# Sur091/GPU-Ray-Tracing

Hardware: AMD Instinct MI355X
Metric: Mrays/s at 1920×1080 (1/2/4/8 GPUs); achieved HBM GB/s vs roofline (higher is better)
Workload: dtype f32; 1 GPU; K3 configs[2]: 1920x1080, 500 spheres, 1 spp, one progressive update per step, max_depth 1; width=1920, height=1080, spheres=500, max_depth=1, parallelism=stripes1, scan=culled, kernel=rt_tpair_kernel<2>, frame_launch=chain

## Files before the change

### gpu-ray-tracing_amd/csrc/rt_abi.cpp

```cpp
#include <hip/hip_runtime_api.h>

#include <algorithm>
#include <cmath>
#include <cstring>
#include <new>
#include <string>
#include <vector>

#include "rt_adaptive.h"
#include "rt_chain_parts.h"
#include "rt_internal.h"
#include "rt_kernels.h"
#include "rt_occlusion_cull.h"
#include "rt_selftest_roots.h"

namespace {
thread_local std::string g_last_error = "";
}

namespace rti {

rt_status fail(rt_status s, const std::string& msg) {
    g_last_error = msg;
    return s;
}

rt_status hip_fail(hipError_t e, const char* what) {
    return fail(RT_ERR_HIP, std::string(what) + ": " + hipGetErrorString(e));
}

constexpr uint32_t kMaxDim = 1u << 16;

rt_status check_image(uint32_t w, uint32_t h) {
    if (w == 0 || h == 0 || w > kMaxDim || h > kMaxDim)
        return fail(RT_ERR_INVALID_SIZE, "image size out of range (1..65536 per side)");
// ... 117 lines not shown
    ctx->occlusion_cull = on != 0;
    return RT_OK;
}

rt_status rt_occlusion_cull_stats(rt_ctx* ctx, uint64_t out[2]) {
    if (!ctx) return fail(RT_ERR_INVALID_CONTEXT, "ctx is NULL");
    if (!out) return fail(RT_ERR_INVALID_ARGUMENT, "out is NULL");
    out[0] = out[1] = 0;
    if (!ctx->cand || ctx->cand_live == 0) return RT_OK;
    DeviceGuard guard(ctx->device);
    if (!guard.ok) return fail(RT_ERR_INVALID_DEVICE, "hipSetDevice failed");
    std::vector<uint32_t> head(2 * ctx->cand_live);
    hipError_t e = hipDeviceSynchronize();
    if (e == hipSuccess)
        e = hipMemcpy2D(head.data(), 2 * sizeof(uint32_t), ctx->cand,
                        rtk::kCandStride * sizeof(float4), 2 * sizeof(uint32_t), ctx->cand_live,
                        hipMemcpyDeviceToHost);
    if (e != hipSuccess) return hip_fail(e, "hipMemcpy2D(candidate counts)");
    for (uint64_t t = 0; t < ctx->cand_live; ++t) {
        if (head[2 * t] == rtk::kCandNone) continue;
        out[0] += head[2 * t + 1];
        out[1] += head[2 * t + 1] ? 1u : 0u;
    }
    return RT_OK;
}

rt_status rt_create(int device, rt_ctx** out_ctx) {
    if (!out_ctx) return fail(RT_ERR_INVALID_ARGUMENT, "out_ctx is NULL");
    *out_ctx = nullptr;
    int n = 0;
    hipError_t e = hipGetDeviceCount(&n);
    if (e != hipSuccess) return hip_fail(e, "hipGetDeviceCount");
    if (device < 0 || device >= n) return fail(RT_ERR_INVALID_DEVICE, "no such HIP device");
    rt_ctx* ctx = new (std::nothrow) rt_ctx();
    if (!ctx) return fail(RT_ERR_NO_MEMORY, "out of host memory");
    ctx->device = device;
    *out_ctx = ctx;
    return RT_OK;
}

rt_status rt_destroy(rt_ctx* ctx) {
    if (!ctx) return fail(RT_ERR_INVALID_CONTEXT, "ctx is NULL");
    rt_status st = RT_OK;
    {
        DeviceGuard guard(ctx->device);
        if (ctx->d_geom || ctx->d_sph || ctx->cand) (void)hipDeviceSynchronize();
// ... 396 lines not shown
```

### gpu-ray-tracing_amd/csrc/rt_context.h

```cpp
#pragma once

#include <hip/hip_runtime_api.h>

#include <vector>

#include "rt_abi.h"

namespace rtc {
struct Chain;
}

struct rt_ctx {
    int device = 0;
    int scan_mode = RT_SCAN_CULLED;
    float4* d_geom = nullptr;
    float4* d_sph = nullptr;
    uint32_t capacity = 0;
    uint32_t count = 0;
    bool valid = false;
    std::vector<rt_sphere> cached;
    uint64_t scene_gen = 0;
    double scene_bound = 0.0;
    bool radii_ok = true;
    bool normal_rn = false;
    uint32_t* d_flag = nullptr;
    float4* d_hint_rs = nullptr;
    void* d_grid = nullptr;
    struct Grid {
        uint32_t nx = 0, nz = 0, nbig = 0, items = 0;
        float x0, z0, s, inv_s, ylo, yhi, cx, cy, cz, reach, m, e;
    } grid;
    float4* cand = nullptr;
    uint32_t* wg_buf = nullptr;
    uint64_t wg_cap = 0;
    uint32_t wg_pix = 0;
    uint32_t wg_parts = 0;
    uint64_t wg_builds = 0;
    uint64_t band_gen = ~0ull, band_seen_gen = ~0ull;
    uint64_t cand_tiles = 0;
    uint64_t cand_live = 0;
    std::vector<unsigned char> cand_key;
    uint64_t cand_gen = 0;
    bool occlusion_cull = true;
    uint32_t* tile_cost = nullptr;
    uint32_t* tile_order = nullptr;
    uint64_t order_tiles = 0;
    uint64_t chain_raster_key[2] = {0, 0};
    uint64_t cost_gen = ~0ull;
    uint32_t cost_frames = 0;
    uint64_t order_gen = ~0ull;
    uint32_t order_frames = 0;
    uint32_t cost_group = 1;
    uint32_t cost_key[6] = {};
    bool cost_key_ok = false;
    uint32_t* d_band_src = nullptr;
    std::vector<uint32_t> band_src;
    int tile_order_mode = RT_TILE_ORDER_AUTO;
    float* d_srgb = nullptr;
    uint32_t* d_hx = nullptr;
    uint32_t hx_len = 0, hy_len = 0;
    struct CountRecord {
        const void* image;
        uint32_t w, h, first, step, bands, n;
    };
    std::vector<CountRecord> counts;
    uint32_t frames_per_launch = 0;
// ... 32 lines not shown
```

### gpu-ray-tracing_amd/csrc/rt_frames.cpp

```cpp
#include <hip/hip_runtime_api.h>

#include <algorithm>
#include <cstdio>
#include <cstdlib>
#include <string>
#include <vector>

#include "rt_chain_parts.h"
#include "rt_internal.h"
#include "rt_kernels.h"
#ifdef RT_CALL_STAMPS
#include <chrono>
static thread_local unsigned long long g_call_stamp[8];
static void call_stamp(int i) {
    g_call_stamp[i] = (unsigned long long)std::chrono::duration_cast<std::chrono::nanoseconds>(
                          std::chrono::steady_clock::now().time_since_epoch())
                          .count();
}
#define CALL_STAMP(i) call_stamp(i)
#else
#define CALL_STAMP(i) ((void)0)
#endif

rt_status rti::chain_report(rt_ctx* ctx) {
// ... 36 lines not shown
    return RT_OK;
}

rt_status join_aux(rt_ctx* ctx, uint32_t n, hipStream_t stream) {
    hipError_t e = hipSuccess;
    for (uint32_t k = 0; e == hipSuccess && k < n; ++k) {
        e = hipEventRecord(ctx->join_ev[k], ctx->aux[k]);
        if (e == hipSuccess) e = hipStreamWaitEvent(stream, ctx->join_ev[k], 0);
    }
    return e == hipSuccess ? RT_OK : hip_fail(e, "join (hipEventRecord / hipStreamWaitEvent)");
}

void note_launch(rt_ctx* ctx, const rtk::TraceParams& p, int kernel, uint32_t frames,
                 uint32_t parts = 1u, bool aql = false) {
    ctx->last.launches += parts;
    ctx->last.queues = parts;
    ctx->last.submit = aql ? RT_SUBMIT_AQL : RT_SUBMIT_HIP;
    ctx->last.frames += frames;
    ctx->last.max_frames_per_launch = std::max(ctx->last.max_frames_per_launch, frames);
    ctx->last.normal_rn = p.normal_rn;
    ctx->last.kernel = kernel != rtk::kTraceBounce ? kernel
                       : p.compact == 3u             ? RT_KERNEL_BOUNCE_SPLIT
                                                     : RT_KERNEL_BOUNCE + (int)p.compact;
}

#ifndef RT_AQL_AUTO_MIN_TILES
#define RT_AQL_AUTO_MIN_TILES 0
#endif
#ifndef RT_AQL_AUTO_MAX_TILES
#define RT_AQL_AUTO_MAX_TILES 0
#endif
constexpr uint64_t kAqlAutoMinTiles = RT_AQL_AUTO_MIN_TILES,
                   kAqlAutoMaxTiles = RT_AQL_AUTO_MAX_TILES;
rt_status usable_chain(rt_ctx* ctx, const rtk::TraceParams& p, rtc::Chain** out) {
    *out = nullptr;
    if (ctx->update_submit == RT_SUBMIT_HIP || ctx->chain_reported) return RT_OK;
    if (ctx->update_submit == RT_SUBMIT_AUTO) {
        const uint64_t tiles = launch_tiles(p.width, p.local_bands);
        if (tiles < kAqlAutoMinTiles || tiles >= kAqlAutoMaxTiles) return RT_OK;
    }
    const bool aql = ctx->update_submit == RT_SUBMIT_AQL;
    if (!ctx->chain_tried) {
        ctx->chain_tried = true;
        rt_status st = RT_OK;
        ctx->chain = rtc::chain_create(ctx->device, &st);
        if (st != RT_OK && aql) return st;
// ... 533 lines not shown
```

### gpu-ray-tracing_amd/csrc/rt_kernels.h

```cpp
#pragma once

#include <hip/hip_runtime_api.h>
#include <stdint.h>

#include "rt_abi.h"

namespace rtk {

constexpr uint32_t kMaxFramesPerLaunch = 128;
constexpr uint32_t kLdsMaxRecords = 4096;
constexpr uint32_t kCandStride = 64;
constexpr uint32_t kCandMax = 19;
constexpr uint32_t kCandRecOff = 1;
constexpr uint32_t kCandSphOff = 21;
constexpr uint32_t kCandNone = 0xFFFFFFFFu;
static_assert(kCandRecOff + ((kCandMax + 3u) & ~3u) <= kCandSphOff, "record chunks fit");
static_assert(kCandSphOff + 2u * kCandMax <= kCandStride, "sphere records fit");
#ifndef RT_HINT_FRAMES
#define RT_HINT_FRAMES 64
#endif
constexpr uint32_t kHintFrames = RT_HINT_FRAMES;
constexpr uint32_t kHintEntries = RT_HINT_FRAMES;
constexpr uint32_t kHintRsDepth = 16;

struct TraceParams {
    const float4* in;
    float4* out;
    float4* out2;
    uint32_t store_each;
    const float4* geom;
    const float4* sph;
    uint32_t width, height, count;
    uint32_t band_first, band_step, local_bands;
    uint32_t frames;
    uint32_t reset_first;
    uint32_t lds_records;
    uint32_t cand_k;
    const float4* cand;
// ... 62 lines not shown
    return k == kTraceListPair || k == kTraceListQuad;
}
constexpr bool is_list_kernel(int k) { return k == kTraceList || is_group_kernel(k); }
#ifndef RT_WG_WAVES
#define RT_WG_WAVES 4
#endif
constexpr bool trace_ordered(int k) {
    return k == kTraceListQuad2 || k == kTraceListPair2 ||
           (is_list_kernel(k) && (is_group_kernel(k) || RT_WG_WAVES == 1));
}
constexpr uint64_t kQuadMaxTiles = 6144;
constexpr uint64_t kQuad2MaxTiles = 20000;
constexpr uint32_t hy_offset(uint32_t width) { return (width + 63u) & ~63u; }
constexpr uint32_t pack_bands(uint32_t first, uint32_t step, bool ordered) {
    return first | ((step < 0x7FFFu ? step : 0x7FFFu) << 16) | (ordered ? 1u << 31 : 0u);
}
hipError_t launch_trace(const TraceParams& p, int kernel, hipStream_t stream);
void arm_launch_events(hipEvent_t start, hipEvent_t stop);
uint32_t disarm_launch_events();
hipError_t launch_deinterleave_bands(const float4* gathered, float4* out, uint32_t width,
                                     uint32_t height, const uint32_t* band_src,
                                     hipStream_t stream);
hipError_t launch_init(float4* out, uint64_t texels, hipStream_t stream);
hipError_t launch_candidates(const TraceParams& p, float4* cand, bool occlusion,
                             hipStream_t stream);
hipError_t launch_wg_order(const float4* cand, uint32_t tiles_x, uint32_t bands, uint32_t pix,
                           uint32_t* wg_cost, uint32_t* wg_order, hipStream_t stream,
                           uint32_t parts);
inline void part_range(uint32_t n, uint32_t parts, uint32_t k, uint32_t& first, uint32_t& len) {
    first = k * (n / parts) + (k < n % parts ? k : n % parts);
    len = n / parts + (k < n % parts ? 1u : 0u);
}
uint32_t single_wg_tiles(uint32_t pix);
uint32_t single_pix();
constexpr int kChainPix1 = 0, kChainPix1Reset = 1, kChainPix = 2, kChainPixReset = 3,
              kChainGo = 4, kChainDone = 5, kChainKernels = 6;
constexpr uint32_t kHiddenArgsBytes = 256;
hipError_t chain_load_kernels();
const char* chain_kernel_symbol(int which);
uint32_t chain_args(const TraceParams& p, int kernel, const uint32_t* abort, unsigned char* out,
                    uint32_t cap, uint32_t grid[2], uint32_t* group_threads, int* which);
hipError_t launch_deinterleave(const float4* gathered, float4* out, uint32_t width,
                               uint32_t height, uint32_t nranks, uint32_t max_local_rows,
                               hipStream_t stream);
hipError_t launch_present(const float4* in, uchar4* out, uint64_t texels,
                          const float* srgb_t, hipStream_t stream);
struct AovParams {
// ... 53 lines not shown
```

### gpu-ray-tracing_amd/csrc/rt_kernels.hip

```cpp
#include <hip/hip_ext.h>
#include <hip/hip_runtime.h>

#include "rt_device.h"
#include "rt_kernels.h"

#include <cstddef>
#include <cstring>

#if defined(__HIP_DEVICE_COMPILE__) && !defined(__gfx950__)
#error "rt_kernels.hip targets gfx950 only (cache-policy bits of the sc1 hand-offs)"
#endif

namespace rtk {

using namespace rtd;

#ifndef RT_WAVE_TRACE
#define RT_WAVE_TRACE 0
#endif
#if RT_WAVE_TRACE
constexpr uint32_t kTraceWaves = 1u << 18;
__device__ unsigned long long g_wave_t[kTraceWaves][2];
__device__ unsigned g_wave_id[kTraceWaves][2];
__device__ __forceinline__ void wave_trace(int end) {
// ... 523 lines not shown
                    black[s] = blk_s;
                } else if (hit[s]) {
                    cf[s] = att;
                    dsky[s] = nd;
                    ddsky[s] = ndd;
                    black[s] = blk_s;
                }
            }
        }
    }
#pragma unroll
    for (uint32_t s = 0; s < S; ++s) {
        const v3 c = sky_w(cf[s], dsky[s], ddsky[s]);
        if (!any_other[s]) {
            asm volatile("");
            col[s] = c;
        } else {
            col[s] = black[s] ? mk(0.0f, 0.0f, 0.0f) : c;
        }
    }
    SST_V(5, col[S - 1].x);
}

template <int kPix, bool kReset, bool kChain>
__device__ __forceinline__ void single_body(
    const float4* __restrict__ a_cand, const uint32_t* __restrict__ a_hx,
    const float4* __restrict__ a_in, uint32_t a_width, uint32_t a_height, uint32_t a_bands,
    const uint32_t* __restrict__ a_order, const SingleParams& p) {
    static_assert(kPix >= 1 && kPix <= 4, "1 to 4 tiles per wave");
    constexpr uint32_t S = kPix;
    WAVE_TRACE(0);
#if RT_SSTAMPS
    sst_put(8, __builtin_amdgcn_s_memrealtime());
    sst_put(0, __builtin_amdgcn_s_memtime());
#endif
    const uint32_t lane = threadIdx.x & 63u;
    const uint32_t wave = __builtin_amdgcn_readfirstlane(threadIdx.x >> 6);
    const uint32_t tiles_x = (a_width + 7u) >> 3;
    const uint32_t aborted =
        kChain ? __builtin_amdgcn_readfirstlane(
                     __hip_atomic_load(p.abort, __ATOMIC_RELAXED, __HIP_MEMORY_SCOPE_SYSTEM))
               : 0u;
    uint32_t gx = blockIdx.x, lband = (p.lbands & 0xFFFFu) + blockIdx.y * (p.lbands >> 16);
    if (a_order) {
        const uint32_t pos = blockIdx.y * (kChain ? p.grid_x : gridDim.x) + blockIdx.x;
        const uint32_t e = __builtin_amdgcn_readfirstlane(a_order[pos]);
// ... 228 lines not shown
template <int G>
__global__ __launch_bounds__(64 * G, RT_TPAIR_MIN_WAVES) void rt_tpair_kernel(
    const float4* __restrict__ a_cand, const uint32_t* __restrict__ a_hx,
    const float4* __restrict__ a_in, uint32_t a_width, uint32_t a_height, uint32_t a_bands,
    const TraceParams p) {
    WAVE_TRACE(0);
    constexpr uint32_t S = 2, Gu = (uint32_t)G;
    static_assert(!kSingleLds<S>, "the pair sample reads its records from the candidate blocks");
    const uint32_t lane = threadIdx.x & 63u;
    const uint32_t w = __builtin_amdgcn_readfirstlane(threadIdx.x >> 6);
    const uint32_t tiles_x = (a_width + 7u) >> 3;
    const uint32_t units_x = (tiles_x + S - 1u) / S;
    uint32_t ux = blockIdx.x, lband = blockIdx.y;
    const uint32_t band_first = a_bands & 0xFFFFu, band_step = (a_bands >> 16) & 0x7FFFu;
    if (a_bands >> 31) {
        const uint32_t t =
            __builtin_amdgcn_readfirstlane(p.tile_order[blockIdx.y * gridDim.x + blockIdx.x]);
        ux = t & 0xFFFFu;
        lband = t >> 16;
    }
    const uint32_t unit = lband * units_x + ux;
    const uint32_t tx0 = ux * S;
    TileCoord tc[S];
    uint32_t ncand[S], hxy[S], tile[S];
    const float4* blk[S];
    float4 acc[S];
    uint64_t valid_m[S];
#pragma unroll
    for (uint32_t s = 0; s < S; ++s) {
        const uint32_t tx = tx0 + s;
        const bool in = tx < tiles_x;
        tile[s] = lband * tiles_x + (in ? tx : tx0);
        tc[s] = tile_coord(a_width, a_height, band_first, band_step, tx, lband, lane);
        blk[s] = a_cand + (size_t)tile[s] * kCandStride;
        ncand[s] = in ? load_cnt(a_cand, tile[s]) : 0u;
        acc[s] = a_in[tc[s].valid ? tc[s].idx : 0];
        hxy[s] = a_hx[min(tc[s].x, a_width - 1u)] ^
                 a_hx[hy_offset(a_width) + min(tc[s].y, a_height - 1u)];
        valid_m[s] = mask_ult(tc[s].x, a_width) & mask_ult(tc[s].y, a_height);
    }
    if (p.tile_cost && w == 0u && lane == 0u)
        p.tile_cost[unit] = (uint32_t)__builtin_amdgcn_s_memtime();
    const Cam cam = cam_params(p);
    const uint32_t n0 = p.hint_n[0];
    if (!p.reset_first &&
        rt_ballot((tc[0].valid && f2u(acc[0].w) != n0) || (tc[1].valid && f2u(acc[1].w) != n0)) !=
            0ull) {
        if (w < S && tx0 + w < tiles_x) {
            const float4 res = trace_pixel<kTraceListQuad, false>(
                p, cam, w ? tile[1] : tile[0], w ? ncand[1] : ncand[0], w ? tc[1] : tc[0],
                w ? hxy[1] : hxy[0], w ? acc[1] : acc[0]);
            const TileCoord& t = w ? tc[1] : tc[0];
            if (t.valid && !p.store_each) p.out[t.idx] = res;
        }
    } else {
        const uint32_t spp = p.spp;
        __shared__ float4 s_cols[2u * Gu * S * 64u];
        __shared__ float4 s_acc[S * 64u];
        if (w == 0u)
#pragma unroll
            for (uint32_t s = 0; s < S; ++s)
                s_acc[s * 64u + lane] = p.reset_first ? make_float4(0.0f, 0.0f, 0.0f, 0.0f)
                                                      : acc[s];
        const float4 zero4 = make_float4(0.0f, 0.0f, 0.0f, 0.0f);
        static_assert(kCandMax < 0x80u && kCandNone == 0xFFFFFFFFu, "a count fits a signed byte");
        const uint32_t unit_state =
            (ncand[0] & 0xFFu) | (ncand[1] & 0xFFu) << 8 | (tile[1] - tile[0]) << 16;
        for (uint32_t f = 0; f < p.frames; f += Gu) {
            const uint32_t fw = f + w;
            v3 col[S];
            const uint32_t ng = fw < p.frames ? p.hint_n[fw] : spp;
            if (ng >= spp) {
#pragma unroll
                for (uint32_t s = 0; s < S; ++s) col[s] = zero_v3_here();
            } else {
                {
                    FrameView v;
                    v.geom = p.geom;
                    v.sph = p.sph;
                    v.count = p.count;
                    v.depth = p.depth;
                    v.seed_b = p.seed_b[fw];
                    v.normal_rn = p.normal_rn;
                    v.rs = p.hint_rs[fw * p.depth];
                    uint32_t seed[S];
                    bool live[S];
                    const float4 bv[S] = {zero4, zero4};
#pragma unroll
                    for (uint32_t s = 0; s < S; ++s) {
                        seed[s] = 1u + ng + v.seed_b;
                        live[s] = tc[s].valid;
                    }
                    const float4* blkf[S];
                    uint32_t ncf[S];
                    uint32_t t0 = tile[0], st = unit_state;
                    asm volatile("" : "+s"(t0), "+s"(st));
#pragma unroll
                    for (uint32_t s = 0; s < S; ++s) {
                        const uint32_t t = t0 + (s ? st >> 16 : 0u);
                        blkf[s] = a_cand + (size_t)t * kCandStride;
                        ncf[s] = (uint32_t)((int32_t)(st << (24u - 8u * s)) >> 24);
                    }
                    single_sample<S, true>(v, cam, tc, hxy, seed, blkf, ncf, live, valid_m, bv,
                                           nullptr, col);
                }
            }
            float4* slot = s_cols + ((f / Gu) & 1u) * Gu * S * 64u;
#pragma unroll
            for (uint32_t t = 0; t < S; ++t)
                if (w != t)
                    *reinterpret_cast<f3v*>(&slot[(w * S + t) * 64u + lane]) =
                        f3v{col[t].x, col[t].y, col[t].z};
            __syncthreads();
#pragma unroll
            for (uint32_t t = 0; t < S; ++t) {
                if (w != t) continue;
#pragma unroll
                for (uint32_t j = 0; j < Gu; ++j) {
                    const uint32_t fj = f + j;
                    if (fj >= p.frames) break;
                    const uint32_t nb = p.hint_n[fj];
                    const bool acc_frame = nb < spp;
                    const float cnt = p.hint_cnt[fj];
                    float4* out = (fj & 1u) ? p.out2 : p.out;
                    const bool store = p.store_each == 2u || fj + 2u >= p.frames;
                    const float4 ca = s_acc[t * 64u + lane];
                    v3 cs = mk(ca.x, ca.y, ca.z);
// ... 691 lines not shown
        __syncthreads();
        for (uint32_t j = lane; j < m; j += 64u) {
            const uint32_t i = s_idx[j];
            s_sph[2u * j] = gsph[2u * i];
            s_sph[2u * j + 1u] = gsph[2u * i + 1u];
        }
        __syncthreads();
        for (uint32_t j = 0; j < m; ++j) {
            const float4 gj = s_rec[j];
            if (ok && !cone_misses(k, gj)) {
                if (n < K) {
                    rec[n] = gj;
                    s_own[n][lane] = gj;
                    sph[2u * n] = s_sph[2u * j];
                    sph[2u * n + 1u] = s_sph[2u * j + 1u];
                }
                ++n;
            }
        }
        __syncthreads();
    }
    if (!mine) return;
    uint32_t removed = 0;
    if (occl && ok && n <= K && n >= 2u) {
        const Lens lens = bundle_lens(p, k);
        float t_occ = __builtin_inff();
        uint32_t j_occ = kCandNone;
        for (uint32_t j = 0; j < n; ++j) {
            const OccBounds b = occ_bounds(k, lens, s_own[j][lane]);
            s_lo[j][lane] = b.lo;
            if (b.covers && b.hi < t_occ) {
                t_occ = b.hi;
                j_occ = j;
            }
        }
        if (j_occ != kCandNone) {
            uint32_t m = 0;
            for (uint32_t j = 0; j < n; ++j) {
                if (j != j_occ && s_lo[j][lane] > t_occ) continue;
                if (m != j) {
                    rec[m] = s_own[j][lane];
                    sph[2u * m] = sph[2u * j];
                    sph[2u * m + 1u] = sph[2u * j + 1u];
                }
                ++m;
            }
            removed = n - m;
            n = m;
        }
    }
    const uint32_t c = ok && n <= K ? n : kCandNone;
    if (c != kCandNone)
        for (uint32_t q = n; q < ((n + 3u) & ~3u); ++q)
            rec[q] = make_float4(0.0f, 0.0f, 0.0f, 0.0f);
    own[0] = make_float4(__uint_as_float(c), __uint_as_float(removed), 0.0f, 0.0f);
}

__global__ __launch_bounds__(256) void rt_init_kernel(float4* __restrict__ out, uint64_t n) {
    const float4 z = make_float4(0.0f, 0.0f, 0.0f, 0.0f);
    for (uint64_t i = (uint64_t)blockIdx.x * blockDim.x + threadIdx.x; i < n;
         i += (uint64_t)gridDim.x * blockDim.x)
        out[i] = z;
}

__global__ __launch_bounds__(256) void rt_deinterleave_kernel(const float4* __restrict__ g,
                                                              float4* __restrict__ out,
                                                              uint32_t width, uint32_t height,
                                                              uint32_t nranks,
                                                              uint32_t max_local_rows) {
    const uint64_t total = (uint64_t)width * height;
    for (uint64_t i = (uint64_t)blockIdx.x * blockDim.x + threadIdx.x; i < total;
         i += (uint64_t)gridDim.x * blockDim.x) {
        const uint32_t y = (uint32_t)(i / width);
        const uint32_t x = (uint32_t)(i - (uint64_t)y * width);
        const uint32_t band = y / RT_STRIPE_ROWS;
        const uint32_t rank = band % nranks;
        const uint32_t lrow = (band / nranks) * RT_STRIPE_ROWS + (y % RT_STRIPE_ROWS);
        out[i] = g[((uint64_t)rank * max_local_rows + lrow) * width + x];
// ... 336 lines not shown
    grid[0] = g.x;
    grid[1] = g.y;
    *group_threads = 64u * kSingleWg;
    *which = (one ? kChainPix1 : kChainPix) + (p.reset_first ? 1 : 0);
    return total;
}

hipError_t launch_trace(const TraceParams& p, int kernel, hipStream_t stream) {
    if (kernel == kTraceSingle) return launch_single<(int)kSinglePix>(p, stream);
    if (kernel == kTraceSingleOne) return launch_single<1>(p, stream);
    if (kernel == kTraceCulled)
        return launch_trace_as<kTraceCulled>(p, (size_t)p.lds_records * sizeof(float4), stream);
    if (kernel == kTraceList) return launch_trace_as<kTraceList>(p, 0, stream);
    if (kernel == kTraceListPair)
        return launch_trace_as<kTraceListPair>(p, group_lds_bytes<kTraceListPair>(), stream);
    if (kernel == kTraceBounce) return launch_bounce(p, stream);
    if (kernel == kTraceListQuad)
        return launch_trace_as<kTraceListQuad>(p, group_lds_bytes<kTraceListQuad>(), stream);
    if (kernel == kTraceListQuad2) return launch_tpair<4>(p, stream);
    if (kernel == kTraceListPair2) return launch_tpair<2>(p, stream);
    return launch_trace_as<kTraceExhaustive>(p, 0, stream);
}

hipError_t launch_candidates(const TraceParams& p, float4* cand, bool occlusion,
                             hipStream_t stream) {
    const uint32_t tiles_x = (p.width + 7u) >> 3;
    const dim3 grid((tiles_x + kCandBX - 1u) / kCandBX,
                    (p.local_bands + kCandBY - 1u) / kCandBY);
    if (grid.x == 0 || grid.y == 0) return hipSuccess;
    hipLaunchKernelGGL(rt_candidates_kernel, grid, dim3(64), 0, stream, p, cand,
                       occlusion ? 1u : 0u);
    return hipGetLastError();
}

uint32_t single_wg_tiles(uint32_t pix) { return kSingleWg * pix; }
uint32_t single_pix() { return kSinglePix; }

hipError_t launch_wg_order(const float4* cand, uint32_t tiles_x, uint32_t bands, uint32_t pix,
                           uint32_t* wg_cost, uint32_t* wg_order, hipStream_t stream,
                           uint32_t parts) {
    const uint32_t per = kSingleWg * pix;
    const uint32_t cols = (tiles_x + per - 1u) / per;
    const uint32_t units = cols * bands;
    if (units == 0) return hipSuccess;
    hipLaunchKernelGGL(rt_wg_cost_kernel, dim3((units + 255u) / 256u), dim3(256), 0, stream, cand,
                       tiles_x, cols, per, units, wg_cost);
    hipError_t e = hipGetLastError();
    if (e != hipSuccess) return e;
    return launch_tile_order(wg_cost, wg_order, units, cols, stream, parts);
}

hipError_t launch_init(float4* out, uint64_t texels, hipStream_t stream) {
    if (texels == 0) return hipSuccess;
    uint64_t blocks = (texels + 255u) / 256u;
// ... 101 lines not shown
```

### gpu-ray-tracing_amd/csrc/rt_occlusion.h

```cpp
#pragma once

#include "rt_trace_device.h"

namespace rtk {

__device__ __forceinline__ v3 cross3(v3 a, v3 b) {
    return mk(a.y * b.z - a.z * b.y, a.z * b.x - a.x * b.z, a.x * b.y - a.y * b.x);
}
__device__ __forceinline__ float l1(v3 v) { return fabsf(v.x) + fabsf(v.y) + fabsf(v.z); }

struct Lens {
    v3 ctr;
    float rl;
};
__device__ __forceinline__ Lens bundle_lens(const TraceParams& p, const Cone& k) {
    Lens b;
    b.ctr = mk(p.center[0], p.center[1], p.center[2]);
    float rl = 0.0f;
    if (p.defocus_angle > 0.0f) {
        const v3 du = mk(p.ddu[0], p.ddu[1], p.ddu[2]), dv = mk(p.ddv[0], p.ddv[1], p.ddv[2]);
        rl = __builtin_amdgcn_sqrtf(dot(du, du) + dot(dv, dv));
    }
    b.rl = rl * 1.001f + 1e-5f * (l1(k.apex) + l1(b.ctr));
    return b;
}

struct OccBounds {
    float lo, hi;
    bool covers;
};
__device__ __forceinline__ OccBounds occ_bounds(const Cone& k, const Lens& b, float4 g) {
    OccBounds r;
    r.lo = -__builtin_inff();
    r.hi = __builtin_inff();
    r.covers = false;
    const v3 C = mk(g.x, g.y, g.z);
    const float R2 = g.w, R = __builtin_amdgcn_sqrtf(g.w);
    const v3 v = sub(C, k.apex);
    const float at = fabsf(dot(v, k.axis)), p = len3(cross3(v, k.axis));
    const float sl = 1e-5f * (at + p + k.r_o) + 1e-6f * (l1(C) + l1(k.apex));
    const float dl_hi = p + at * k.sin_t + k.r_o + sl;
    const float dl_lo = fmaf(p, k.cos_t, -at * k.sin_t) - k.r_o - sl;
    const v3 w = sub(C, b.ctr);
    const float D = len3(w), tc = dot(w, k.axis), pc = len3(cross3(w, k.axis));
    const float sd = 1e-5f * D + 1e-6f * (l1(C) + l1(b.ctr));
    const float s_hi = D + b.rl + sd, s_lo = D - b.rl - sd;
    const bool ahead = tc * k.cos_t - pc * k.sin_t - b.rl - sd > 0.0f && s_lo > R * 1.0001f;
    if (!ahead || !__builtin_isfinite(s_hi + dl_hi + R)) return r;
    const float E = 2e-6f * fmaf(s_hi, s_hi, R2);
    const float q2 = R2 - dl_hi * dl_hi;
    const bool inside = q2 > E;
    const float err = 1e-6f * (s_hi + R) +
                      (inside ? E * __builtin_amdgcn_rsqf(q2) * 1.0001f
                              : __builtin_amdgcn_sqrtf(E) * 1.0001f);
    {
        const float dl = fminf(fmaxf(dl_lo, 0.0f), R);
        const float num = (s_lo - R) * (s_lo + R);
        const float den = __builtin_amdgcn_sqrtf(fmaf(-dl, dl, s_lo * s_lo) * 1.000001f +
                                                 1e-6f * s_lo * s_lo) +
                          __builtin_amdgcn_sqrtf(fmaxf(fmaf(-dl, dl, R2), 0.0f) + 1e-6f * R2);
        r.lo = num / den * 0.9999f - err;
    }
    if (inside) {
        const float num = (s_hi - R) * (s_hi + R);
        const float den =
            __builtin_amdgcn_sqrtf(fmaxf(fmaf(-dl_hi, dl_hi, s_hi * s_hi) - 1e-6f * s_hi * s_hi,
                                         0.0f)) +
            __builtin_amdgcn_sqrtf(fmaxf(q2 - 1e-6f * R2, 0.0f));
        const float tangent = __builtin_amdgcn_sqrtf(num);
        r.hi = fminf(num / den, tangent) * 1.0001f + err;
        r.covers = s_lo - R - err > 1.1e-3f * k.d_max && __builtin_isfinite(r.hi);
    }
    return r;
}

}
```

### gpu-ray-tracing_amd/csrc/rt_plan.cpp

```cpp
#include <hip/hip_runtime_api.h>

#include <algorithm>
#include <cmath>
#include <cstdlib>
#include <cstring>
#include <vector>

#include "rt_device.h"
#include "rt_internal.h"
#include "rt_kernels.h"

namespace rti {

int trace_kernel_for(const rt_ctx* ctx, const rtk::TraceParams& p) {
    if (ctx->scan_mode == RT_SCAN_EXHAUSTIVE) return rtk::kTraceExhaustive;
#ifndef RT_FORCE_CULLED_KERNEL
    if (p.depth <= 1u && camera_rays_bounded(ctx, p)) return rtk::kTraceList;
#endif
#ifndef RT_NO_BOUNCE_KERNEL
    if (p.depth >= 2u) return rtk::kTraceBounce;
#endif
    return rtk::kTraceCulled;
}

// ... 27 lines not shown
                                    (tpair && tiles <= rtk::kQuad2MaxTiles)));
    return quad ? (tpair ? rtk::kTraceListQuad2 : rtk::kTraceListQuad)
                : (tpair ? rtk::kTraceListPair2 : rtk::kTraceListPair);
}

UnitGrid frame_group_units(int kernel, uint32_t w, uint32_t bands) {
    const uint32_t group =
        kernel == rtk::kTraceListQuad2 || kernel == rtk::kTraceListPair2 ? 2u : 1u;
    const uint32_t units_x = (((w + 7u) >> 3) + group - 1u) / group;
    return {group, units_x, (uint64_t)units_x * bands};
}

void free_candidates(rt_ctx* ctx) {
    (void)hipFree(ctx->cand);
    ctx->cand = nullptr;
    ctx->cand_tiles = 0;
    ctx->cand_live = 0;
    ctx->cand_key.clear();
}

static rt_status ensure_candidates(rt_ctx* ctx, rtk::TraceParams& p, hipStream_t stream) {
    struct Key {
        float center[3], vul[3], pdu[3], pdv[3], ddu[3], ddv[3], defocus;
        uint32_t w, h, first, step, bands, occlusion;
        uint64_t scene;
    } key;
    std::memset(&key, 0, sizeof(key));
    std::memcpy(key.center, p.center, sizeof(key.center));
    std::memcpy(key.vul, p.vul, sizeof(key.vul));
    std::memcpy(key.pdu, p.pdu, sizeof(key.pdu));
    std::memcpy(key.pdv, p.pdv, sizeof(key.pdv));
    std::memcpy(key.ddu, p.ddu, sizeof(key.ddu));
    std::memcpy(key.ddv, p.ddv, sizeof(key.ddv));
    key.defocus = p.defocus_angle;
    key.w = p.width;
    key.h = p.height;
    key.first = p.band_first;
    key.step = p.band_step;
    key.bands = p.local_bands;
    key.scene = ctx->scene_gen;
    const bool occlusion = ctx->occlusion_cull && ctx->scene_bound <= 0x1p40 &&
                           camera_rays_bounded(ctx, p);
    key.occlusion = occlusion ? 1u : 0u;
    const unsigned char* kb = reinterpret_cast<const unsigned char*>(&key);
    const uint64_t tiles = launch_tiles(p.width, p.local_bands);
    p.cand_k = rtk::kCandMax;
    if (ctx->cand_key.size() != sizeof(key) ||
        std::memcmp(ctx->cand_key.data(), kb, sizeof(key)) != 0) {
        if (tiles > ctx->cand_tiles) {
            if (ctx->cand_tiles) {
                hipError_t e = hipStreamSynchronize(stream);
                if (e != hipSuccess) return hip_fail(e, "hipStreamSynchronize");
            }
            free_candidates(ctx);
            hipError_t e = hipMalloc(&ctx->cand, tiles * rtk::kCandStride * sizeof(float4));
            if (e != hipSuccess) {
                free_candidates(ctx);
                return hip_fail(e, "hipMalloc(candidate lists)");
            }
            ctx->cand_tiles = tiles;
        }
        hipError_t e = rtk::launch_candidates(p, ctx->cand, occlusion, stream);
        if (e != hipSuccess) return hip_fail(e, "rt_candidates_kernel launch");
        ctx->cand_key.assign(kb, kb + sizeof(key));
        ctx->cand_gen++;
        ctx->cand_live = tiles;
    }
    p.cand = ctx->cand;
    return RT_OK;
}

rt_status ensure_order_buffers(rt_ctx* ctx, uint64_t tiles, hipStream_t stream) {
    if (tiles <= ctx->order_tiles) return RT_OK;
    if (ctx->order_tiles) {
        hipError_t e = hipStreamSynchronize(stream);
        if (e != hipSuccess) return hip_fail(e, "hipStreamSynchronize");
    }
    (void)hipFree(ctx->tile_cost);
    (void)hipFree(ctx->tile_order);
    ctx->tile_cost = ctx->tile_order = nullptr;
    ctx->order_tiles = 0;
    ctx->cost_gen = ctx->order_gen = ~0ull;
    ctx->chain_raster_key[0] = 0;
    hipError_t e = hipMalloc(&ctx->tile_cost, tiles * sizeof(uint32_t));
    if (e == hipSuccess) e = hipMalloc(&ctx->tile_order, 3 * tiles * sizeof(uint32_t));
// ... 415 lines not shown
```

### gpu-ray-tracing_amd/gpu_ray_tracing/_lib.py

```python
from __future__ import annotations

import ctypes
import os
from pathlib import Path

import torch

PKG_ROOT = Path(__file__).resolve().parent.parent
LIB_PATH = PKG_ROOT / "build" / "librt_hip.so"

F = ctypes.c_float
U32 = ctypes.c_uint32


class RtError(RuntimeError):

    def __init__(self, status: int, func: str, message: str):
        super().__init__(f"{func} failed with status {status} ({STATUS_NAMES.get(status, '?')}): "
                         f"{message}")
        self.status = status


STATUS_NAMES = {
    0: "RT_OK",
# ... 97 lines not shown
    "rt_comm_group_start": (ctypes.c_int, []),
    "rt_comm_group_end": (ctypes.c_int, []),
    "rt_gather_stripes": (ctypes.c_int, [P, P, P, P, P, U32, U32, U32, P]),
    "rt_update_frames_bands": (ctypes.c_int, [P, P, P, U32, U32, P, P, P, U32, U32, P, P,
                                              ctypes.POINTER(ctypes.c_int)]),
    "rt_band_costs": (ctypes.c_int, [P, U32, U32, P, P]),
    "rt_partition_bands": (ctypes.c_int, [P, U32, U32, P]),
    "rt_deinterleave_bands": (ctypes.c_int, [P, P, P, U32, U32, U32, P, U32, P]),
    "rt_gather_bands": (ctypes.c_int, [P, P, P, P, P, U32, U32, P, U32, P]),
    "rt_set_launch_timing": (ctypes.c_int, [P, ctypes.c_int]),
    "rt_last_call_kernel_time": (ctypes.c_int, [P, ctypes.POINTER(F), ctypes.POINTER(U32)]),
}

_SIGS_CHAIN_PARTS = {
    "rt_set_chain_parts": (ctypes.c_int, [P, U32]),
    "rt_chain_schedule": (ctypes.c_int, [U32, U32, ctypes.c_int, P, U32, ctypes.POINTER(U32)]),
}

_SIGS_OCCLUSION = {
    "rt_set_occlusion_cull": (ctypes.c_int, [P, ctypes.c_int]),
    "rt_occlusion_cull_stats": (ctypes.c_int, [P, P]),
}

_SIGS_SELFTEST_ROOTS = {
    "rt_selftest_roots": (ctypes.c_int, [P, ctypes.c_uint64, P]),
}
RT_ROOTS_FAMILIES = 2
RT_ROOTS_STRATA = 4

_SIGS_AOV = {
    "rt_trace_aov": (ctypes.c_int, [P, P, U32, U32, P, P, U32, P]),
    "rt_trace_aov_bands": (ctypes.c_int, [P, P, U32, U32, P, P, P, U32, P]),
    "rt_pick": (ctypes.c_int, [P, U32, U32, U32, U32, P, P, U32, P, P]),
}
RT_AOV_MISS = 0xFFFFFFFF
AOV_PLANES = ("sphere_id", "hit", "normal", "material")


class AovPlanesC(ctypes.Structure):
    _fields_ = [("sphere_id", P), ("hit", P), ("normal", P), ("material", P)]


class PickResultC(ctypes.Structure):
    _fields_ = [("sphere_id", U32), ("t", F), ("p", F * 3), ("normal", F * 3),
                ("front_face", U32), ("color", F * 4)]

# ... 170 lines not shown
    _fields_ = [("part", U32), ("first", U32), ("frames", U32)]


class RootsTallyC(ctypes.Structure):
    _fields_ = [("mismatches", ctypes.c_uint64), ("drawn", ctypes.c_uint64),
                ("compared", ctypes.c_uint64), ("rooted", ctypes.c_uint64)]


_lib = None


def lib() -> ctypes.CDLL:
    global _lib
    if _lib is None:
        path = Path(os.environ.get("RT_HIP_LIB", LIB_PATH))
        if not path.exists():
            raise RuntimeError(f"librt_hip.so not found at {path}: build it with "
                               f"`make -C {PKG_ROOT}` (no CPU fallback exists)")
        handle = ctypes.CDLL(str(path))
        for name, (res, args) in {**_SIGS, **_SIGS_CHAIN_PARTS, **_SIGS_SELFTEST_ROOTS,
                                  **_SIGS_AOV, **_SIGS_DENOISE, **_SIGS_REPROJECT,
                                  **_SIGS_VARIANCE, **_SIGS_ADAPTIVE, **_SIGS_CONVERGE,
                                  **_SIGS_PROGRESS, **_SIGS_EDIT, **_SIGS_OCCLUSION,
                                  **_SIGS_MATTE, **_SIGS_QUERY}.items():
            if "RT_HIP_LIB" in os.environ and not hasattr(handle, name):
                continue
            fn = getattr(handle, name)
            fn.restype = res
            fn.argtypes = args
        _lib = handle
    return _lib


_fast = False


def fastcall():
    global _fast
    if _fast is False:
        _fast = None
        if "RT_HIP_LIB" not in os.environ:
            import importlib.machinery
            import importlib.util
            import sysconfig
            path = PKG_ROOT / "build" / ("_rt_fastcall" + sysconfig.get_config_var("EXT_SUFFIX"))
            if path.exists():
                lib()
                loader = importlib.machinery.ExtensionFileLoader("_rt_fastcall", str(path))
                spec = importlib.util.spec_from_file_location("_rt_fastcall", path,
                                                              loader=loader)
                mod = importlib.util.module_from_spec(spec)
                loader.exec_module(mod)
                _fast = mod
    return _fast


def exported_symbols() -> list[str]:
    return list(_SIGS)


def chain_parts_symbols() -> list[str]:
    return list(_SIGS_CHAIN_PARTS)


def occlusion_symbols() -> list[str]:
    return list(_SIGS_OCCLUSION)


def selftest_roots_symbols() -> list[str]:
    return list(_SIGS_SELFTEST_ROOTS)


def aov_symbols() -> list[str]:
    return list(_SIGS_AOV)


def denoise_symbols() -> list[str]:
    return list(_SIGS_DENOISE)


def reproject_symbols() -> list[str]:
    return list(_SIGS_REPROJECT)


def variance_symbols() -> list[str]:
    return list(_SIGS_VARIANCE)


def adaptive_symbols() -> list[str]:
    return list(_SIGS_ADAPTIVE)

# ... 30 lines not shown
```

### gpu-ray-tracing_amd/gpu_ray_tracing/compute_shader.py

```python
from __future__ import annotations

import ctypes

import numpy as np
import torch

from . import _lib
from .camera import SceneCamera
from .scene import SphereCollection

RT_STRIPE_ROWS = _lib.RT_STRIPE_ROWS
DENOISE_DEFAULTS = {"iterations": 5, "normal_power_log2": 5, "sigma_color": 1.0,
                    "sigma_position": 0.5}


REPROJECT_DEFAULTS = {"max_history": 64, "position_tolerance2": 1e-5, "lambertian_only": True}


GUIDED_DEFAULTS = {"iterations": 5, "normal_power_log2": 5, "sigma_luminance": 1.0,
                   "sigma_position": 0.5, "min_history": 4, "fallback_variance": 1.0}


ADAPTIVE_DEFAULTS = {"min_samples": 16, "abs_tolerance2": 1e-5, "rel_tolerance2": 2.5e-4}

# ... 136 lines not shown
            self._ctx = ctypes.c_void_p()

    def set_frames_per_launch(self, n: int) -> None:
        _lib.call("rt_set_frames_per_launch", self._ctx, int(n))

    def set_frame_pairs(self, mode: str) -> None:
        _lib.call("rt_set_frame_pairs", self._ctx,
                  {"auto": 0, "off": 1, "on": 2, "quad": 3, "on2": 4, "quad2": 5}[mode])

    def set_frame_images(self, mode: str) -> None:
        _lib.call("rt_set_frame_images", self._ctx, {"last_two": 0, "every": 1}[mode])

    def set_tile_order(self, mode: str) -> None:
        _lib.call("rt_set_tile_order", self._ctx, {"auto": 0, "off": 1}[mode])

    def set_update_queues(self, queues: int) -> None:
        _lib.call("rt_set_update_queues", self._ctx, int(queues))

    def set_chain_parts(self, parts: int) -> None:
        _lib.call("rt_set_chain_parts", self._ctx, int(parts))

    def set_occlusion_cull(self, on: bool) -> None:
        _lib.call("rt_set_occlusion_cull", self._ctx, 1 if on else 0)

    def set_update_submit(self, mode: str) -> None:
        _lib.call("rt_set_update_submit", self._ctx, {"auto": 0, "hip": 1, "aql": 2}[mode])

    def submit_status(self) -> dict:
        avail, give_ups, packets = ctypes.c_int(0), _lib.U32(0), ctypes.c_uint64(0)
        _lib.call("rt_update_submit_status", self._ctx, ctypes.byref(avail),
                  ctypes.byref(give_ups), ctypes.byref(packets))
        why = "" if avail.value else _lib.lib().rt_last_error().decode()
        return {"aql_available": bool(avail.value), "go_give_ups": int(give_ups.value),
                "packets": int(packets.value), "why": why}

    def set_path_compaction(self, mode: str) -> None:
        _lib.call("rt_set_path_compaction", self._ctx,
                  {"auto": 0, "per_wave": 1, "compact": 2, "pair": 3, "split": 4}[mode])

    def set_single_kernel(self, mode: str) -> None:
        _lib.call("rt_set_single_kernel", self._ctx,
                  {"auto": 0, "off": 1, "pair": 2, "one": 3}[mode])

    def frames_per_launch(self, camera) -> int:
        out = _lib.U32(0)
        cam = camera.to_c()
# ... 843 lines not shown
```

Before: 201,800 Mrays/s.

## Add certain-tile fast path skipping candidate intersection loop in pair kernel

The candidate builder now flags 8-pixel tiles where exactly one sphere remains after occlusion culling and that sphere provably covers every ray in the tile. It stores a tile-certain bit plus a material class in the tile header. The pair trace kernel packs these flags into its per-unit state. When both tiles of a pair are certain, it uses a specialised sampler that intersects that one sphere directly and shades by material class, bypassing the general candidate loop and its hit tests. This costs an extra flag load, more kernel code and registers, and a stricter coverage test in the candidate kernel. It also adds a toggle and a stats query.

```diff
diff --git a/gpu-ray-tracing_amd/csrc/rt_abi.cpp b/gpu-ray-tracing_amd/csrc/rt_abi.cpp
--- a/gpu-ray-tracing_amd/csrc/rt_abi.cpp
+++ b/gpu-ray-tracing_amd/csrc/rt_abi.cpp
@@ -11,6 +11,7 @@
 #include "rt_chain_parts.h"
 #include "rt_internal.h"
 #include "rt_kernels.h"
+#include "rt_certain_tiles.h"
 #include "rt_occlusion_cull.h"
 #include "rt_selftest_roots.h"
 
@@ -174,6 +175,37 @@
         out[0] += head[2 * t + 1];
         out[1] += head[2 * t + 1] ? 1u : 0u;
     }
+    return RT_OK;
+}
+
+rt_status rt_set_certain_tiles(rt_ctx* ctx, int on) {
+    if (!ctx) return fail(RT_ERR_INVALID_CONTEXT, "ctx is NULL");
+    if (on != 0 && on != 1) return fail(RT_ERR_INVALID_ARGUMENT, "on must be 0 or 1");
+    ctx->certain_tiles = on != 0;
+    return RT_OK;
+}
+
+rt_status rt_certain_tiles_stats(rt_ctx* ctx, uint64_t out[2]) {
+    if (!ctx) return fail(RT_ERR_INVALID_CONTEXT, "ctx is NULL");
+    if (!out) return fail(RT_ERR_INVALID_ARGUMENT, "out is NULL");
+    out[0] = out[1] = 0;
+    if (!ctx->cand || ctx->cand_live == 0 || ctx->scan_mode != RT_SCAN_CULLED) return RT_OK;
+    DeviceGuard guard(ctx->device);
+    if (!guard.ok) return fail(RT_ERR_INVALID_DEVICE, "hipSetDevice failed");
+    std::vector<uint32_t> flags(ctx->cand_live);
+    hipError_t e = hipDeviceSynchronize();
+    if (e == hipSuccess)
+        e = hipMemcpy2D(flags.data(), sizeof(uint32_t),
+                        reinterpret_cast<const uint32_t*>(ctx->cand) + 2,
+                        rtk::kCandStride * sizeof(float4), sizeof(uint32_t), ctx->cand_live,
+                        hipMemcpyDeviceToHost);
+    if (e != hipSuccess) return hip_fail(e, "hipMemcpy2D(tile flags)");
+    for (uint32_t f : flags) out[0] += f & rtk::kTileCertain;
+    const uint64_t tx = ctx->pair_tiles_x;
+    if (ctx->pair_gen == ctx->cand_gen && tx * ctx->pair_bands == ctx->cand_live)
+        for (uint64_t b = 0; b < ctx->pair_bands; ++b)
+            for (uint64_t x = 0; x + 1 < tx; x += 2)
+                out[1] += flags[b * tx + x] & flags[b * tx + x + 1] & rtk::kTileCertain;
     return RT_OK;
 }
 
diff --git a/gpu-ray-tracing_amd/csrc/rt_context.h b/gpu-ray-tracing_amd/csrc/rt_context.h
--- a/gpu-ray-tracing_amd/csrc/rt_context.h
+++ b/gpu-ray-tracing_amd/csrc/rt_context.h
@@ -42,6 +42,9 @@
     std::vector<unsigned char> cand_key;
     uint64_t cand_gen = 0;
     bool occlusion_cull = true;
+    bool certain_tiles = true;
+    uint64_t pair_gen = ~0ull;
+    uint32_t pair_tiles_x = 0, pair_bands = 0;
     uint32_t* tile_cost = nullptr;
     uint32_t* tile_order = nullptr;
     uint64_t order_tiles = 0;
diff --git a/gpu-ray-tracing_amd/csrc/rt_frames.cpp b/gpu-ray-tracing_amd/csrc/rt_frames.cpp
--- a/gpu-ray-tracing_amd/csrc/rt_frames.cpp
+++ b/gpu-ray-tracing_amd/csrc/rt_frames.cpp
@@ -82,6 +82,11 @@
     ctx->last.kernel = kernel != rtk::kTraceBounce ? kernel
                        : p.compact == 3u             ? RT_KERNEL_BOUNCE_SPLIT
                                                      : RT_KERNEL_BOUNCE + (int)p.compact;
+    if (kernel == rtk::kTraceListPair2 || kernel == rtk::kTraceListQuad2) {
+        ctx->pair_gen = ctx->cand_gen;
+        ctx->pair_tiles_x = (p.width + 7u) >> 3;
+        ctx->pair_bands = p.local_bands;
+    }
 }
 
 #ifndef RT_AQL_AUTO_MIN_TILES
diff --git a/gpu-ray-tracing_amd/csrc/rt_kernels.h b/gpu-ray-tracing_amd/csrc/rt_kernels.h
--- a/gpu-ray-tracing_amd/csrc/rt_kernels.h
+++ b/gpu-ray-tracing_amd/csrc/rt_kernels.h
@@ -14,6 +14,8 @@
 constexpr uint32_t kCandRecOff = 1;
 constexpr uint32_t kCandSphOff = 21;
 constexpr uint32_t kCandNone = 0xFFFFFFFFu;
+constexpr uint32_t kTileCertain = 1u;
+constexpr uint32_t kClassLambertian = 0u, kClassMetal = 1u, kClassDielectric = 2u;
 static_assert(kCandRecOff + ((kCandMax + 3u) & ~3u) <= kCandSphOff, "record chunks fit");
 static_assert(kCandSphOff + 2u * kCandMax <= kCandStride, "sphere records fit");
 #ifndef RT_HINT_FRAMES
@@ -122,7 +124,7 @@
                                      uint32_t height, const uint32_t* band_src,
                                      hipStream_t stream);
 hipError_t launch_init(float4* out, uint64_t texels, hipStream_t stream);
-hipError_t launch_candidates(const TraceParams& p, float4* cand, bool occlusion,
+hipError_t launch_candidates(const TraceParams& p, float4* cand, bool occlusion, bool certain,
                              hipStream_t stream);
 hipError_t launch_wg_order(const float4* cand, uint32_t tiles_x, uint32_t bands, uint32_t pix,
                            uint32_t* wg_cost, uint32_t* wg_order, hipStream_t stream,
diff --git a/gpu-ray-tracing_amd/csrc/rt_kernels.hip b/gpu-ray-tracing_amd/csrc/rt_kernels.hip
--- a/gpu-ray-tracing_amd/csrc/rt_kernels.hip
+++ b/gpu-ray-tracing_amd/csrc/rt_kernels.hip
@@ -569,6 +569,94 @@
     SST_V(5, col[S - 1].x);
 }
 
+__device__ __forceinline__ uint32_t load_flags(const float4* cand, uint32_t tile) {
+    return ((const kconst uint32_t*)cand)[(size_t)tile * (4u * kCandStride) + 2u];
+}
+
+template <typename P>
+__device__ __forceinline__ void certain_sample(const P& p, const Cam& cam,
+                                               const TileCoord (&tc)[2],
+                                               const uint32_t (&hxy)[2],
+                                               const uint32_t (&seed)[2],
+                                               const float4* const (&blk)[2],
+                                               const uint32_t (&cls)[2], const bool (&live)[2],
+                                               const uint64_t (&live_m)[2], v3 (&col)[2]) {
+    constexpr uint32_t S = 2;
+    v3 o[S], d[S];
+    v3 c0 = cam.center;
+    asm volatile("" : "+v"(c0.x), "+v"(c0.y), "+v"(c0.z));
+#pragma unroll
+    for (uint32_t s = 0; s < S; ++s)
+        get_ray<kSingleDisk>(cam, tc[s].x, tc[s].y, hxy[s], seed[s] * 25u + p.seed_b, o[s],
+                             d[s], &c0);
+    asm volatile("" ::"v"(c0.x), "v"(c0.y), "v"(c0.z));
+    if (flag_here(p, p.depth) == 0u) {
+#pragma unroll
+        for (uint32_t s = 0; s < S; ++s)
+            col[s] = sky_w(mk(1.0f, 1.0f, 1.0f), d[s], dot(d[s], d[s]));
+        return;
+    }
+    const float r_sb = p.rs.x;
+    const v3 ruv = mk(p.rs.y, p.rs.z, p.rs.w);
+#pragma unroll
+    for (uint32_t s = 0; s < S; ++s) {
+        const float a = dot(d[s], d[s]);
+        const float4 g = load_rec<true>(blk[s] + kCandRecOff, 0);
+        const float4 pr = load_rec<true>(blk[s] + kCandSphOff, 0);
+        const float4 mat = load_rec<true>(blk[s] + kCandSphOff, 1);
+        float h;
+        const float disc = discriminant(g, o[s], d[s], a, h);
+        const float q = sqrt_core(disc + 0x1p-126f);
+        const float t = div_core(h - q, a, rcp_refined(a));
+        const v3 hp = fmas(t, d[s], o[s]);
+        const v3 rel = sub(hp, mk(pr.x, pr.y, pr.z));
+        v3 n;
+        if ((__builtin_amdgcn_fcmpf(min_abs3(rel), 0x1p-100f, 4) & live_m[s]) == 0ull) {
+            const float y = rcp_refined(pr.w);
+            n = normal_div(rel, pr.w, y, flag_here(p, p.normal_rn) != 0u);
+        } else {
+            n = divs(rel, pr.w);
+        }
+        const v3 att = mk(mat.x, mat.y, mat.z);
+        if (cls[s] == kClassLambertian) {
+            v3 dir = add(n, ruv);
+            float ndd = dot(dir, dir);
+            if ((__builtin_amdgcn_fcmpf(ndd, 0x1.0c6f7ap-20f, 4) & live_m[s]) != 0ull) {
+                asm volatile("");
+                if (ndd < 0x1.0c6f7ap-20f) {
+                    dir = n;
+                    ndd = dot(n, n);
+                }
+            }
+            col[s] = sky_w(att, dir, ndd);
+        } else {
+            v3 nd = d[s], cf = att;
+            float ndd = a;
+            bool black = false;
+            if (live[s]) {
+                if (cls[s] == kClassMetal) {
+                    const v3 refl = fmas(mat.w, ruv, normalize_w<true>(reflect(d[s], n)));
+                    black = !(dot(refl, n) > 0.0f);
+                    nd = normalize_w<true>(refl);
+                    ndd = dot(nd, nd);
+                } else {
+                    cf = mk(1.0f, 1.0f, 1.0f);
+                    const float ratio = 1.0f / mat.x;
+                    const v3 u = normalize_w<true>(d[s]);
+                    const float cos_t = fminf(dot(neg(u), n), 1.0f);
+                    const float sin_t = sqrtf(fmaf(-cos_t, cos_t, 1.0f));
+                    const bool cannot = ratio * sin_t > 1.0f;
+                    const bool refl = cannot || reflectance(cos_t, ratio) > r_sb;
+                    nd = normalize_w<true>(refl ? reflect(u, n) : refract(u, n, ratio));
+                    ndd = dot(nd, nd);
+                }
+            }
+            const v3 c = sky_w(cf, nd, ndd);
+            col[s] = black ? mk(0.0f, 0.0f, 0.0f) : c;
+        }
+    }
+}
+
 template <int kPix, bool kReset, bool kChain>
 __device__ __forceinline__ void single_body(
     const float4* __restrict__ a_cand, const uint32_t* __restrict__ a_hx,
@@ -843,7 +931,7 @@
     const uint32_t unit = lband * units_x + ux;
     const uint32_t tx0 = ux * S;
     TileCoord tc[S];
-    uint32_t ncand[S], hxy[S], tile[S];
+    uint32_t ncand[S], hxy[S], tile[S], tflags[S];
     const float4* blk[S];
     float4 acc[S];
     uint64_t valid_m[S];
@@ -855,6 +943,7 @@
         tc[s] = tile_coord(a_width, a_height, band_first, band_step, tx, lband, lane);
         blk[s] = a_cand + (size_t)tile[s] * kCandStride;
         ncand[s] = in ? load_cnt(a_cand, tile[s]) : 0u;
+        tflags[s] = in ? load_flags(a_cand, tile[s]) : 0u;
         acc[s] = a_in[tc[s].valid ? tc[s].idx : 0];
         hxy[s] = a_hx[min(tc[s].x, a_width - 1u)] ^
                  a_hx[hy_offset(a_width) + min(tc[s].y, a_height - 1u)];
@@ -886,7 +975,9 @@
         const float4 zero4 = make_float4(0.0f, 0.0f, 0.0f, 0.0f);
         static_assert(kCandMax < 0x80u && kCandNone == 0xFFFFFFFFu, "a count fits a signed byte");
         const uint32_t unit_state =
-            (ncand[0] & 0xFFu) | (ncand[1] & 0xFFu) << 8 | (tile[1] - tile[0]) << 16;
+            (ncand[0] & 0xFFu) | (ncand[1] & 0xFFu) << 8 | (tile[1] - tile[0]) << 16 |
+            (tflags[0] & 7u) << 24 | (tflags[1] & 7u) << 27;
+        constexpr uint32_t kPairCertain = kTileCertain << 24 | kTileCertain << 27;
         for (uint32_t f = 0; f < p.frames; f += Gu) {
             const uint32_t fw = f + w;
             v3 col[S];
@@ -918,12 +1009,17 @@
                     asm volatile("" : "+s"(t0), "+s"(st));
 #pragma unroll
                     for (uint32_t s = 0; s < S; ++s) {
-                        const uint32_t t = t0 + (s ? st >> 16 : 0u);
+                        const uint32_t t = t0 + (s ? (st >> 16) & 1u : 0u);
                         blkf[s] = a_cand + (size_t)t * kCandStride;
                         ncf[s] = (uint32_t)((int32_t)(st << (24u - 8u * s)) >> 24);
                     }
-                    single_sample<S, true>(v, cam, tc, hxy, seed, blkf, ncf, live, valid_m, bv,
-                                           nullptr, col);
+                    if ((st & kPairCertain) == kPairCertain) {
+                        const uint32_t cls[S] = {(st >> 25) & 3u, (st >> 28) & 3u};
+                        certain_sample(v, cam, tc, hxy, seed, blkf, cls, live, valid_m, col);
+                    } else {
+                        single_sample<S, true>(v, cam, tc, hxy, seed, blkf, ncf, live, valid_m,
+                                               bv, nullptr, col);
+                    }
                 }
             }
             float4* slot = s_cols + ((f / Gu) & 1u) * Gu * S * 64u;
@@ -1661,16 +1757,19 @@
     }
     if (!mine) return;
     uint32_t removed = 0;
-    if (occl && ok && n <= K && n >= 2u) {
+    bool front_one = false;
+    if ((occl & 1u) && ok && n <= K && n >= 2u) {
         const Lens lens = bundle_lens(p, k);
         float t_occ = __builtin_inff();
         uint32_t j_occ = kCandNone;
         for (uint32_t j = 0; j < n; ++j) {
-            const OccBounds b = occ_bounds(k, lens, s_own[j][lane]);
+            const float4 gj = s_own[j][lane];
+            const OccBounds b = occ_bounds(k, lens, gj);
             s_lo[j][lane] = b.lo;
             if (b.covers && b.hi < t_occ) {
                 t_occ = b.hi;
                 j_occ = j;
+                front_one = certainly_front(b, gj);
             }
         }
         if (j_occ != kCandNone) {
@@ -1687,12 +1786,22 @@
             removed = n - m;
             n = m;
         }
+    } else if (occl == 3u && ok && n == 1u && n <= K) {
+        const float4 g = s_own[0][lane];
+        front_one = certainly_front(occ_bounds(k, bundle_lens(p, k), g), g);
+    }
+    uint32_t flags = 0;
+    if ((occl & 2u) && ok && n <= K && n == 1u && front_one) {
+        const float radius = sph[0].w, matw = sph[1].w;
+        if (radius > 0.0f && __builtin_isfinite(radius))
+            flags = kTileCertain | material_class(matw) << 1;
     }
     const uint32_t c = ok && n <= K ? n : kCandNone;
     if (c != kCandNone)
         for (uint32_t q = n; q < ((n + 3u) & ~3u); ++q)
             rec[q] = make_float4(0.0f, 0.0f, 0.0f, 0.0f);
-    own[0] = make_float4(__uint_as_float(c), __uint_as_float(removed), 0.0f, 0.0f);
+    own[0] = make_float4(__uint_as_float(c), __uint_as_float(removed), __uint_as_float(flags),
+                         0.0f);
 }
 
 __global__ __launch_bounds__(256) void rt_init_kernel(float4* __restrict__ out, uint64_t n) {
@@ -2075,14 +2184,14 @@
     return launch_trace_as<kTraceExhaustive>(p, 0, stream);
 }
 
-hipError_t launch_candidates(const TraceParams& p, float4* cand, bool occlusion,
+hipError_t launch_candidates(const TraceParams& p, float4* cand, bool occlusion, bool certain,
                              hipStream_t stream) {
     const uint32_t tiles_x = (p.width + 7u) >> 3;
     const dim3 grid((tiles_x + kCandBX - 1u) / kCandBX,
                     (p.local_bands + kCandBY - 1u) / kCandBY);
     if (grid.x == 0 || grid.y == 0) return hipSuccess;
     hipLaunchKernelGGL(rt_candidates_kernel, grid, dim3(64), 0, stream, p, cand,
-                       occlusion ? 1u : 0u);
+                       occlusion ? (certain ? 3u : 1u) : 0u);
     return hipGetLastError();
 }
 
diff --git a/gpu-ray-tracing_amd/csrc/rt_occlusion.h b/gpu-ray-tracing_amd/csrc/rt_occlusion.h
--- a/gpu-ray-tracing_amd/csrc/rt_occlusion.h
+++ b/gpu-ray-tracing_amd/csrc/rt_occlusion.h
@@ -28,12 +28,14 @@
 struct OccBounds {
     float lo, hi;
     bool covers;
+    float q2, err;
 };
 __device__ __forceinline__ OccBounds occ_bounds(const Cone& k, const Lens& b, float4 g) {
     OccBounds r;
     r.lo = -__builtin_inff();
     r.hi = __builtin_inff();
     r.covers = false;
+    r.q2 = r.err = 0.0f;
     const v3 C = mk(g.x, g.y, g.z);
     const float R2 = g.w, R = __builtin_amdgcn_sqrtf(g.w);
     const v3 v = sub(C, k.apex);
@@ -70,8 +72,20 @@
         const float tangent = __builtin_amdgcn_sqrtf(num);
         r.hi = fminf(num / den, tangent) * 1.0001f + err;
         r.covers = s_lo - R - err > 1.1e-3f * k.d_max && __builtin_isfinite(r.hi);
+        r.q2 = q2;
+        r.err = err;
     }
     return r;
 }
 
+__device__ __forceinline__ bool certainly_front(const OccBounds& b, float4 g) {
+    const float R = __builtin_amdgcn_sqrtf(g.w);
+    return b.covers && 0.9f * __builtin_amdgcn_sqrtf(b.q2) >
+                           2.0f * (b.err + 1e-6f * (l1(mk(g.x, g.y, g.z)) + R));
 }
+
+__device__ __forceinline__ uint32_t material_class(float w) {
+    return w < -1.0f ? kClassLambertian : w <= 1.0f ? kClassMetal : kClassDielectric;
+}
+
+}
diff --git a/gpu-ray-tracing_amd/csrc/rt_plan.cpp b/gpu-ray-tracing_amd/csrc/rt_plan.cpp
--- a/gpu-ray-tracing_amd/csrc/rt_plan.cpp
+++ b/gpu-ray-tracing_amd/csrc/rt_plan.cpp
@@ -73,7 +73,7 @@
 static rt_status ensure_candidates(rt_ctx* ctx, rtk::TraceParams& p, hipStream_t stream) {
     struct Key {
         float center[3], vul[3], pdu[3], pdv[3], ddu[3], ddv[3], defocus;
-        uint32_t w, h, first, step, bands, occlusion;
+        uint32_t w, h, first, step, bands, occlusion, certain;
         uint64_t scene;
     } key;
     std::memset(&key, 0, sizeof(key));
@@ -93,6 +93,8 @@
     const bool occlusion = ctx->occlusion_cull && ctx->scene_bound <= 0x1p40 &&
                            camera_rays_bounded(ctx, p);
     key.occlusion = occlusion ? 1u : 0u;
+    const bool certain = occlusion && ctx->certain_tiles;
+    key.certain = certain ? 1u : 0u;
     const unsigned char* kb = reinterpret_cast<const unsigned char*>(&key);
     const uint64_t tiles = launch_tiles(p.width, p.local_bands);
     p.cand_k = rtk::kCandMax;
@@ -111,7 +113,7 @@
             }
             ctx->cand_tiles = tiles;
         }
-        hipError_t e = rtk::launch_candidates(p, ctx->cand, occlusion, stream);
+        hipError_t e = rtk::launch_candidates(p, ctx->cand, occlusion, certain, stream);
         if (e != hipSuccess) return hip_fail(e, "rt_candidates_kernel launch");
         ctx->cand_key.assign(kb, kb + sizeof(key));
         ctx->cand_gen++;
diff --git a/gpu-ray-tracing_amd/gpu_ray_tracing/_lib.py b/gpu-ray-tracing_amd/gpu_ray_tracing/_lib.py
--- a/gpu-ray-tracing_amd/gpu_ray_tracing/_lib.py
+++ b/gpu-ray-tracing_amd/gpu_ray_tracing/_lib.py
@@ -143,6 +143,11 @@
     "rt_occlusion_cull_stats": (ctypes.c_int, [P, P]),
 }
 
+_SIGS_CERTAIN = {
+    "rt_set_certain_tiles": (ctypes.c_int, [P, ctypes.c_int]),
+    "rt_certain_tiles_stats": (ctypes.c_int, [P, P]),
+}
+
 _SIGS_SELFTEST_ROOTS = {
     "rt_selftest_roots": (ctypes.c_int, [P, ctypes.c_uint64, P]),
 }
@@ -359,7 +364,7 @@
                                   **_SIGS_AOV, **_SIGS_DENOISE, **_SIGS_REPROJECT,
                                   **_SIGS_VARIANCE, **_SIGS_ADAPTIVE, **_SIGS_CONVERGE,
                                   **_SIGS_PROGRESS, **_SIGS_EDIT, **_SIGS_OCCLUSION,
-                                  **_SIGS_MATTE, **_SIGS_QUERY}.items():
+                                  **_SIGS_MATTE, **_SIGS_QUERY, **_SIGS_CERTAIN}.items():
             if "RT_HIP_LIB" in os.environ and not hasattr(handle, name):
                 continue
             fn = getattr(handle, name)
@@ -404,6 +409,10 @@
     return list(_SIGS_OCCLUSION)
 
 
+def certain_symbols() -> list[str]:
+    return list(_SIGS_CERTAIN)
+
+
 def selftest_roots_symbols() -> list[str]:
     return list(_SIGS_SELFTEST_ROOTS)
 
diff --git a/gpu-ray-tracing_amd/gpu_ray_tracing/compute_shader.py b/gpu-ray-tracing_amd/gpu_ray_tracing/compute_shader.py
--- a/gpu-ray-tracing_amd/gpu_ray_tracing/compute_shader.py
+++ b/gpu-ray-tracing_amd/gpu_ray_tracing/compute_shader.py
@@ -182,6 +182,16 @@
 
     def set_occlusion_cull(self, on: bool) -> None:
         _lib.call("rt_set_occlusion_cull", self._ctx, 1 if on else 0)
+
+    def set_certain_tiles(self, on: bool) -> None:
+        if hasattr(_lib.lib(), "rt_set_certain_tiles"):
+            _lib.call("rt_set_certain_tiles", self._ctx, 1 if on else 0)
+
+    def certain_tiles_stats(self) -> dict:
+        out = (ctypes.c_uint64 * 2)()
+        if hasattr(_lib.lib(), "rt_certain_tiles_stats"):
+            _lib.call("rt_certain_tiles_stats", self._ctx, out)
+        return {"certain_tiles": int(out[0]), "certain_pairs": int(out[1])}
 
     def set_update_submit(self, mode: str) -> None:
         _lib.call("rt_set_update_submit", self._ctx, {"auto": 0, "hip": 1, "aql": 2}[mode])
diff --git a/include/rt_certain_tiles.h b/include/rt_certain_tiles.h
--- /dev/null
+++ b/include/rt_certain_tiles.h
@@ -0,0 +1,17 @@
+#ifndef RT_CERTAIN_TILES_H
+#define RT_CERTAIN_TILES_H
+
+#include "rt_abi.h"
+
+#ifdef __cplusplus
+extern "C" {
+#endif
+
+RT_API rt_status rt_set_certain_tiles(rt_ctx* ctx, int on);
+RT_API rt_status rt_certain_tiles_stats(rt_ctx* ctx, uint64_t out[2]);
+
+#ifdef __cplusplus
+}
+#endif
+
+#endif
```

New measurement: 212,000 Mrays/s, median of 6. 5.0% higher.
